# Amandaynzhou/MMT-PSM

Hardware: AMD Instinct MI355X
Metric: imgs/sec (student+teacher step, 1000x1000, AUG_K=2) (higher is better)
Workload: dtype f32

## Files before the change

mmt-psm_amd/csrc/conv_wgpl.hip:

```cpp
#include "conv_shared.h"

namespace {

constexpr unsigned WG_OOB = 0x80000000u;
constexpr int WG_BLK = 1024 + 128;
constexpr int WG_GSTAGE = 32 * WG_BLK;
constexpr int WG_STAGE = 2 * WG_GSTAGE, WG_S = 2;

typedef short s16x4 __attribute__((ext_vector_type(4)));

__device__ __forceinline__ f16x8 tr_pair(const char* p) {
  const s16x4 a = __builtin_amdgcn_ds_read_tr16_b64_v4i16((__attribute__((address_space(3))) s16x4*)(p));
  const s16x4 b = __builtin_amdgcn_ds_read_tr16_b64_v4i16((__attribute__((address_space(3))) s16x4*)(p + 128));
  typedef short s16x8 __attribute__((ext_vector_type(8)));
  const s16x8 v = {a[0], a[1], a[2], a[3], b[0], b[1], b[2], b[3]};
  return __builtin_bit_cast(f16x8, v);
}

struct WgP {
  const float* x; const float* dy;
  const unsigned short* xpl; long xpl_stride;
  const unsigned short* dpl; long dpl_stride;
  const float* s_x; const float* s_dy;
  const float* guard_x; const float* guard_dy;
  const float* rowscale; float* dw; float* ws; float* dbias;
  int N, H, W, Cin, Cout, KH, KW, pad, ksplit;
  int lag;
};

__device__ __forceinline__ void wgrad_pl_body(const WgP& p, const int bid_in, const int nwg_in) {
  extern __shared__ __attribute__((aligned(16))) float lds[];
  char* const ring = (char*)lds;
  const int tid = threadIdx.x, lane = tid & 63;
  const int wave = __builtin_amdgcn_readfirstlane(tid >> 6);
  const bool copier = wave >= 8;
  const int grp = copier ? (wave - 8) >> 1 : wave >> 2;
  const int gw = wave & 3, wm = gw >> 1, wn = gw & 1;
  const int NP = p.KH * p.KW * p.Cin, tiles_n = NP >> 7;
  int bid = bid_in;
  {
    const int nwg = nwg_in, q = nwg >> 3, r = nwg & 7, xcd = bid & 7, idx = bid >> 3;
    bid = (xcd < r ? xcd * (q + 1) : r * (q + 1) + (xcd - r) * q) + idx;
  }
  const int tile = bid % ((p.Cout >> 7) * tiles_n), ks = bid / ((p.Cout >> 7) * tiles_n);
  const int tile_m = tile / tiles_n, tile_n = tile - tile_m * tiles_n;
  const int co0 = tile_m * 128, n0 = tile_n * 128;
  const int tap = n0 / p.Cin, ci0 = n0 - tap * p.Cin;
  const int kh = tap / p.KW, kw = tap - kh * p.KW;
  const int dkh = kh - p.pad, dkw = kw - p.pad;
  const F16Guard gx = f16_guard_load(p.guard_x), gd = f16_guard_load(p.guard_dy);
  const int T = (p.N * p.H * p.W) >> 5, R = 2 * p.ksplit, rng = ks * 2 + grp;
  const int t0 = (int)((long)rng * T / R), nt = (int)((long)(rng + 1) * T / R) - t0;
  const int nt_max = (T + R - 1) / R;
  const int segs = p.W >> 5;
  char* const gring = ring + grp * WG_GSTAGE;

  f32x16 acc[2][2];
#pragma unroll
  for (int a = 0; a < 2; a++)
#pragma unroll
    for (int b = 0; b < 2; b++)
#pragma unroll
      for (int r = 0; r < 16; r++) acc[a][b][r] = 0.f;
  float bsum[2] = {0.f, 0.f};
  const bool do_bias = p.dbias != nullptr && tile_n == 0 && wn == 0 && !copier;
  const bool slow = ((p.lag & 1) ? f16_guard_bad_lag(gx, *p.s_x) : f16_guard_bad(gx)) ||
                    ((p.lag & 2) ? f16_guard_bad_lag(gd, *p.s_dy) : f16_guard_bad(gd));

  if (copier && !slow) {
    const int sub = (wave - 8) & 1;
    const long n_d = (long)p.N * p.H * p.W * p.Cout, n_x = (long)p.N * p.H * p.W * p.Cin;
    const __amdgpu_buffer_rsrc_t rs0 = sub == 0 ? __builtin_amdgcn_make_buffer_rsrc((void*)p.dpl, 0, (int)(n_d * 2), 0x00020000)
                                                : __builtin_amdgcn_make_buffer_rsrc((void*)((const char*)p.xpl - 64), 0, (int)(n_x * 2 + 64), 0x00020000);
    const __amdgpu_buffer_rsrc_t rs1 = sub == 0 ? __builtin_amdgcn_make_buffer_rsrc((void*)(p.dpl + p.dpl_stride), 0, (int)(n_d * 2), 0x00020000)
                                                : __builtin_amdgcn_make_buffer_rsrc((void*)((const char*)(p.xpl + p.xpl_stride) - 64), 0, (int)(n_x * 2 + 64), 0x00020000);
    const int cbn = (sub == 0 ? p.Cout : p.Cin) >> 4;
    const int cb0 = (sub == 0 ? co0 : ci0) >> 4;
    const int px = lane >> 1;
    int f_t = 0;
    auto copy_step = [&](int stage) {
      const bool real = f_t < nt;
      const int t = t0 + (real ? f_t : 0);
      const int row = t / segs, w0 = (t - row * segs) << 5;
      unsigned vo = (unsigned)lane * 16u;
      int soff;
      if (sub == 0) {
        soff = (row * cbn + cb0) * (p.W * 32) + w0 * 32;
        if (!real) vo = WG_OOB;
      } else {
        const int h = row % p.H, ih = h + dkh, iw = w0 + px + dkw;
        const bool ok = real && (unsigned)ih < (unsigned)p.H && (unsigned)iw < (unsigned)p.W;
        soff = ((row + dkh) * cbn + cb0) * (p.W * 32) + (w0 + dkw) * 32 + 64;
        if (!ok) { vo = WG_OOB; }
        if (!(real && (unsigned)ih < (unsigned)p.H)) soff = 64;
      }
      char* const st = gring + stage * WG_STAGE + sub * 16 * WG_BLK;
#pragma unroll
      for (int cb = 0; cb < 8; cb++) {
        __builtin_amdgcn_raw_ptr_buffer_load_lds(rs0, (lds_ptr_t)(st + cb * WG_BLK), 16, (int)vo, soff + cb * (p.W * 32), 0, 0);
        __builtin_amdgcn_raw_ptr_buffer_load_lds(rs1, (lds_ptr_t)(st + (8 + cb) * WG_BLK), 16, (int)vo, soff + cb * (p.W * 32), 0, 0);
      }
      f_t++;
    };
    copy_step(0);
    asm volatile("s_waitcnt vmcnt(0)" ::: "memory");
    __builtin_amdgcn_s_barrier();
    copy_step(1);
    for (int t = 0; t < nt_max; t++) {
      asm volatile("s_waitcnt vmcnt(0)" ::: "memory");
      __builtin_amdgcn_s_barrier();
      copy_step(t & 1);
    }
    asm volatile("s_waitcnt vmcnt(0)" ::: "memory");
  } else if (!slow) {
    const int i16 = lane & 15, g1 = (lane >> 4) & 1, khalf = lane >> 5;
    const int loff = khalf * 256 + (i16 >> 2) * 32 + (i16 & 3) * 8;
    const char* const fA = gring + (wm * 4 + g1) * WG_BLK + loff;
    const char* const fB = gring + (16 + wn * 4 + g1) * WG_BLK + loff;
    __builtin_amdgcn_s_barrier();
    for (int t = 0; t < nt_max; t++) {
      const char* const sa = fA + (t & 1) * WG_STAGE;
      const char* const sb = fB + (t & 1) * WG_STAGE;
      if (t < nt) {
#pragma unroll
        for (int k2 = 0; k2 < 2; k2++) {
          f16x8 fa[2][2], fb[2][2];
#pragma unroll
          for (int q = 0; q < 2; q++)
#pragma unroll
            for (int a = 0; a < 2; a++) {
              fa[q][a] = tr_pair(sa + (q * 8 + a * 2) * WG_BLK + k2 * 512);
              fb[q][a] = tr_pair(sb + (q * 8 + a * 2) * WG_BLK + k2 * 512);
            }
          if (do_bias) {
#pragma unroll
            for (int a = 0; a < 2; a++)
#pragma unroll
              for (int e = 0; e < 8; e++) bsum[a] += (float)fa[0][a][e] + (float)fa[1][a][e];
          }
#pragma unroll
          for (int pr = 0; pr < 3; pr++) {
            const int qa = pr == 1 ? 1 : 0, qb = pr == 0 ? 1 : 0;
#pragma unroll
            for (int a = 0; a < 2; a++)
#pragma unroll
              for (int b = 0; b < 2; b++) acc[a][b] = __builtin_amdgcn_mfma_f32_32x32x16_f16(fa[qa][a], fb[qb][b], acc[a][b], 0, 0, 0);
          }
        }
      }
      asm volatile("s_waitcnt lgkmcnt(0)" ::: "memory");
      __builtin_amdgcn_s_barrier();
    }
  }
  const float sxy = *p.s_x * *p.s_dy;
  if (slow) {
    if (!copier) {
      const int HW = p.H * p.W;
      for (int m = t0 * 32; m < (t0 + nt) * 32; m++) {
        const int img = m / HW, rem = m - img * HW, h = rem / p.W, w = rem - h * p.W;
        const int ih = h + dkh, iw = w + dkw;
        const bool ok = (unsigned)ih < (unsigned)p.H && (unsigned)iw < (unsigned)p.W;
#pragma unroll
        for (int b = 0; b < 2; b++) {
          const float xv = ok ? p.x[((long)(img * p.H + ih) * p.W + iw) * p.Cin + ci0 + wn * 64 + b * 32 + (lane & 31)] : 0.f;
#pragma unroll
          for (int a = 0; a < 2; a++)
#pragma unroll
            for (int r = 0; r < 16; r++) {
              const int co = co0 + wm * 64 + a * 32 + 8 * (r >> 2) + (r & 3) + 4 * (lane >> 5);
              acc[a][b][r] = fmaf(p.dy[(long)m * p.Cout + co], xv, acc[a][b][r]);
            }
        }
        if (do_bias && lane < 32) {
#pragma unroll
          for (int a = 0; a < 2; a++) bsum[a] += p.dy[(long)m * p.Cout + co0 + wm * 64 + a * 32 + lane] * *p.s_dy;
        }
      }
#pragma unroll
      for (int a = 0; a < 2; a++)
#pragma unroll
        for (int b = 0; b < 2; b++)
#pragma unroll
          for (int r = 0; r < 16; r++) acc[a][b][r] *= sxy;
    }
  }
  __syncthreads();

  if (do_bias) {
    const float inv_d = 1.f / *p.s_dy;
#pragma unroll
    for (int a = 0; a < 2; a++) {
      float v = bsum[a];
      if (!slow) v += __shfl_xor(v, 32, 64);
      if (lane < 32) atomicAdd(p.dbias + co0 + wm * 64 + a * 32 + lane, v * inv_d);
    }
  }

  {
    f32x4* const xch = (f32x4*)ring;
    const int gtid = tid & 255;
#pragma unroll
    for (int i = 0; i < 4; i++) {
      if (!copier && (i & 1) != grp) {
#pragma unroll
        for (int r4 = 0; r4 < 4; r4++)
          xch[(i * 4 + r4) * 256 + gtid] = f32x4{acc[i >> 1][i & 1][4 * r4], acc[i >> 1][i & 1][4 * r4 + 1],
                                                 acc[i >> 1][i & 1][4 * r4 + 2], acc[i >> 1][i & 1][4 * r4 + 3]};
      }
    }
    __syncthreads();
#pragma unroll
    for (int i = 0; i < 4; i++) {
      if (!copier && (i & 1) == grp) {
#pragma unroll
        for (int r4 = 0; r4 < 4; r4++) {
          const f32x4 v = xch[(i * 4 + r4) * 256 + gtid];
#pragma unroll
          for (int c = 0; c < 4; c++) {
            const float mine = acc[i >> 1][i & 1][4 * r4 + c];
            acc[i >> 1][i & 1][4 * r4 + c] = grp == 0 ? mine + v[c] : v[c] + mine;
          }
        }
      }
    }
  }
  if (copier) return;

  const float inv = 1.f / sxy;
  float* const dst = p.ksplit > 1 ? p.ws + (long)ks * p.Cout * NP : p.dw;
#pragma unroll
  for (int i = 0; i < 4; i++) {
    if ((i & 1) != grp) continue;
    const int a = i >> 1, b = i & 1;
#pragma unroll
    for (int r = 0; r < 16; r++) {
      const int co = co0 + wm * 64 + a * 32 + 8 * (r >> 2) + (r & 3) + 4 * (lane >> 5);
      float* const q = dst + (long)co * NP + n0 + wn * 64 + b * 32 + (lane & 31);
      if (p.ksplit > 1) *q = acc[a][b][r] * inv;
      else *q = *q + acc[a][b][r] * ((p.rowscale ? p.rowscale[co] : 1.f) * inv);
    }
  }
}

__global__ __launch_bounds__(768) void wgrad_pl_kernel(const WgP p) { wgrad_pl_body(p, blockIdx.x, gridDim.x); }

constexpr int WG_MAXG = 12;
struct WgGroup { WgP it[WG_MAXG]; int first[WG_MAXG + 1]; int n; };
static_assert(sizeof(WgGroup) <= 3584, "kernel-argument segment");
__global__ __launch_bounds__(768) void wgrad_pl_group_kernel(const WgGroup g) {
  int i = 0;
  for (int k = 1; k < g.n; k++) i = (int)blockIdx.x >= g.first[k] ? k : i;
  const int local = (int)blockIdx.x - g.first[i];
  const WgP p = g.it[i];
  const int real = (p.Cout >> 7) * ((p.KH * p.KW * p.Cin) >> 7) * p.ksplit;
  if (local >= real) return;
  wgrad_pl_body(p, local, real);
}

constexpr int WG_MAXR = 24;
struct WgReduceGroup { mmtconv::WgReduceItem it[WG_MAXR]; int first[WG_MAXR + 1]; int n; };
static_assert(sizeof(WgReduceGroup) <= 3584, "kernel-argument segment");
__global__ __launch_bounds__(256) void wgrad_reduce_group_kernel(const WgReduceGroup g) {
  int k = 0;
  for (int j = 1; j < g.n; j++) k = (int)blockIdx.x >= g.first[j] ? j : k;
  const mmtconv::WgReduceItem it = g.it[k];
  const int nb = g.first[k + 1] - g.first[k], lb = (int)blockIdx.x - g.first[k];
  const long n4 = (long)it.Cout * it.NP / 4, slab = (long)it.Cout * it.NP;
  for (long i = (long)lb * 256 + threadIdx.x; i < n4; i += (long)nb * 256) {
    f32x4 o = ((f32x4*)it.dw)[i];
    f32x4 a = ((const f32x4*)it.ws)[i];
    int s = 1;
    for (; s + 8 <= it.splits; s += 8) {
      f32x4 b[8];
#pragma unroll
      for (int u = 0; u < 8; u++) b[u] = *(const f32x4*)(it.ws + (s + u) * slab + i * 4);
#pragma unroll
      for (int u = 0; u < 8; u++) a += b[u];
    }
    for (; s < it.splits; s++) a += *(const f32x4*)(it.ws + s * slab + i * 4);
    const float sc = it.rowscale ? it.rowscale[(int)((i * 4) / it.NP)] : 1.f;
#pragma unroll
    for (int e = 0; e < 4; e++) o[e] += a[e] * sc;
    ((f32x4*)it.dw)[i] = o;
  }
}

__global__ __launch_bounds__(256) void wgrad_pl_reduce_kernel(const float* __restrict__ ws, int splits, int Cout, int NP,
                                                              const float* __restrict__ rowscale, float* __restrict__ dw) {
  const long n4 = (long)Cout * NP / 4, slab = (long)Cout * NP;
  for (long i = (long)blockIdx.x * 256 + threadIdx.x; i < n4; i += (long)gridDim.x * 256) {
    f32x4 o = ((f32x4*)dw)[i];
    f32x4 a = ((const f32x4*)ws)[i];
    int s = 1;
    for (; s + 8 <= splits; s += 8) {
      f32x4 b[8];
#pragma unroll
      for (int u = 0; u < 8; u++) b[u] = *(const f32x4*)(ws + (s + u) * slab + i * 4);
#pragma unroll
      for (int u = 0; u < 8; u++) a += b[u];
    }
    for (; s < splits; s++) a += *(const f32x4*)(ws + s * slab + i * 4);
    const float sc = rowscale ? rowscale[(int)((i * 4) / NP)] : 1.f;
#pragma unroll
    for (int e = 0; e < 4; e++) o[e] += a[e] * sc;
    ((f32x4*)dw)[i] = o;
  }
}

int wgpl_splits(const mmt_conv_args* a) {
  if (precision() != 3 || a->stride != 1 || a->Ho != a->H || a->Wo != a->W || (a->W & 31) || (a->Cin & 127) || (a->Cout & 127) ||
      a->KH != a->KW || a->pad != (a->KH - 1) / 2 || !(a->KH & 1) || a->N < 1 || a->io_bf16 ||
      (long)a->N * a->H * a->W * (a->Cin > a->Cout ? a->Cin : a->Cout) >= (1L << 29))
    return 0;
  const char* e = getenv("MMT_WGRAD_PLANES");
  if (e && atoi(e) == 0) return 0;
  const long T = ((long)a->N * a->H * a->W) >> 5;
  const long tiles = (long)(a->Cout >> 7) * ((long)a->KH * a->KW * a->Cin >> 7);
  constexpr long target = 256;
  long ks = target / tiles;
  if (ks > T / 8) ks = T / 8;
  if (ks < 1) ks = 1;
  if (T < 2) return 0;
  return (int)ks;
}

}

namespace mmtconv {
int wgpl_eligible_splits(const mmt_conv_args* a) { return a ? wgpl_splits(a) : 0; }
long wgpl_super_steps(const mmt_conv_args* a) { return ((long)a->N * a->H * a->W) >> 5; }

int launch_wgrad_reduce_group(const WgReduceItem* items, int n, hipStream_t s) {
  for (int i0 = 0; i0 < n; i0 += WG_MAXR) {
    WgReduceGroup g;
    g.n = n - i0 < WG_MAXR ? n - i0 : WG_MAXR;
    int nb = 0;
    for (int i = 0; i < g.n; i++) {
      g.it[i] = items[i0 + i];
      g.first[i] = nb;
      long b = ((long)items[i0 + i].Cout * items[i0 + i].NP / 4 + 255) / 256;
      nb += (int)(b > 1024 ? 1024 : b);
    }
    g.first[g.n] = nb;
    hipLaunchKernelGGL(wgrad_reduce_group_kernel, dim3(nb), dim3(256), 0, s, g);
    MMT_LAUNCH_CHECK();
  }
  return 0;
}

int launch_wgpl_group(const WgPlJob* jobs, int n, hipStream_t s) {
  if (n < 1 || n > WG_MAXG) return MMT_EINVAL;
  WgGroup g;
  g.n = n;
  int nb = 0;
  for (int i = 0; i < n; i++) {
    const WgPlJob& j = jobs[i];
    const mmt_conv_args* a = j.a;
    if (!a->x || !j.dy || !j.xpl || !j.dpl || !j.s_x || !j.s_dy || !j.dw || ((size_t)j.xpl & 15) || ((size_t)j.dpl & 15) ||
        (j.xpl_stride & 7) || (j.dpl_stride & 7) || j.ksplit < 1 || (j.ksplit > 1 && !j.ws))
      return MMT_EINVAL;
    WgP& p = g.it[i];
    p.x = a->x; p.dy = j.dy;
    p.xpl = (const unsigned short*)j.xpl; p.xpl_stride = j.xpl_stride;
    p.dpl = (const unsigned short*)j.dpl; p.dpl_stride = j.dpl_stride;
    p.s_x = j.s_x; p.s_dy = j.s_dy;
    p.guard_x = (const float*)a->f16_guard_x; p.guard_dy = (const float*)a->f16_guard_dy;
    p.rowscale = j.rowscale; p.dw = j.dw; p.ws = j.ws; p.dbias = j.dbias;
    p.lag = a->x_planes_lag;
    p.N = a->N; p.H = a->H; p.W = a->W; p.Cin = a->Cin; p.Cout = a->Cout; p.KH = a->KH; p.KW = a->KW; p.pad = a->pad; p.ksplit = j.ksplit;
    g.first[i] = nb;
    const int blocks = (a->Cout >> 7) * ((a->KH * a->KW * a->Cin) >> 7) * j.ksplit;
    nb += (blocks + 7) & ~7;
  }
  g.first[n] = nb;
  constexpr size_t lds = (size_t)WG_S * WG_STAGE;
  static bool done = false;
  if (!done) {
    const hipError_t e = hipFuncSetAttribute((const void*)wgrad_pl_group_kernel, hipFuncAttributeMaxDynamicSharedMemorySize, (int)lds);
    if (e != hipSuccess) return (int)e;
    done = true;
  }
  hipLaunchKernelGGL(wgrad_pl_group_kernel, dim3(nb), dim3(768), lds, s, g);
  MMT_LAUNCH_CHECK();
  return 0;
}
}

extern "C" int mmt_conv_wgrad_planes_splits(const mmt_conv_args* a) { return a ? wgpl_splits(a) : 0; }

extern "C" int mmt_conv_wgrad_planes(const mmt_conv_args* a, const float* dy, const void* x_planes, long x_plane_stride,
                                     const void* dy_planes, long dy_plane_stride, const float* s_x, const float* s_dy,
                                     const float* rowscale, float* dw, float* dbias, float* workspace, void* stream) {
  if (!a) return MMT_EINVAL;
  const int ks = wgpl_splits(a);
  if (ks == 0) return 1;
  if (!a->x || !dy || !x_planes || !dy_planes || !s_x || !s_dy || !dw || ((size_t)x_planes & 15) || ((size_t)dy_planes & 15) ||
      (x_plane_stride & 7) || (dy_plane_stride & 7) || (ks > 1 && !workspace))
    return MMT_EINVAL;
  WgP p;
  p.x = a->x; p.dy = dy;
  p.xpl = (const unsigned short*)x_planes; p.xpl_stride = x_plane_stride;
  p.dpl = (const unsigned short*)dy_planes; p.dpl_stride = dy_plane_stride;
  p.s_x = s_x; p.s_dy = s_dy;
  p.guard_x = (const float*)a->f16_guard_x; p.guard_dy = (const float*)a->f16_guard_dy;
  p.rowscale = rowscale; p.dw = dw; p.ws = workspace; p.dbias = dbias;
  p.lag = a->x_planes_lag;
  p.N = a->N; p.H = a->H; p.W = a->W; p.Cin = a->Cin; p.Cout = a->Cout; p.KH = a->KH; p.KW = a->KW; p.pad = a->pad; p.ksplit = ks;
  const int NP = a->KH * a->KW * a->Cin;
  const int tiles = (a->Cout >> 7) * (NP >> 7);
  constexpr size_t lds = (size_t)WG_S * WG_STAGE;
  static_assert(lds <= 160 * 1024 && lds >= 16 * 256 * 16, "LDS");
  static bool done = false;
  if (!done) {
    const hipError_t e = hipFuncSetAttribute((const void*)wgrad_pl_kernel, hipFuncAttributeMaxDynamicSharedMemorySize, (int)lds);
    if (e != hipSuccess) return (int)e;
    done = true;
  }
  hipStream_t s = (hipStream_t)stream;
  hipLaunchKernelGGL(wgrad_pl_kernel, dim3(tiles * ks), dim3(768), lds, s, p);
  MMT_LAUNCH_CHECK();
  if (ks > 1) {
    const long n4 = (long)a->Cout * NP / 4;
    int blocks = (int)((n4 + 255) / 256);
    if (blocks > 4096) blocks = 4096;
    hipLaunchKernelGGL(wgrad_pl_reduce_kernel, dim3(blocks), dim3(256), 0, s, workspace, ks, a->Cout, NP, rowscale, dw);
    MMT_LAUNCH_CHECK();
  }
  return 0;
}
```

mmt-psm_amd/csrc/conv_wgrad.hip:

```cpp
#include <stdlib.h>
#include <type_traits>
#include "conv_shared.h"

namespace {

template <bool FAST>
__global__ __launch_bounds__(256) void conv_wgrad_kernel(const ConvP p, const float* __restrict__ dy,
                                                         const float* __restrict__ rowscale,
                                                         float* __restrict__ dw, int m_per_split,
                                                         float* __restrict__ ws) {
  constexpr int BM = 128, BN = 128;
  extern __shared__ __attribute__((aligned(16))) float lds[];
  float* ldsA = lds;
  float* ldsB = lds + 2 * 32 * 128;
  const int tid = threadIdx.x, lane = tid & 63;
  const int wave = __builtin_amdgcn_readfirstlane(tid >> 6);
  const int wm = wave >> 1, wn = wave & 1;
  const int co0 = blockIdx.y * BM, n0 = blockIdx.x * BN;
  const int NP = p.KH * p.KW * p.Cin;
  const int ms = blockIdx.z * m_per_split;
  const int me = min(p.M, ms + m_per_split);
  if (ms >= me) return;

  const int c4 = tid & 31;
// ... 725 lines not shown
  for (long i = (long)blockIdx.x * 256 + threadIdx.x; i < n4; i += (long)gridDim.x * 256) {
    f32x4 o = ((f32x4*)dw)[i];
    f32x4 a = ((const f32x4*)ws)[i];
    int s = 1;
    for (; s + 8 <= splits; s += 8) {
      f32x4 b[8];
#pragma unroll
      for (int u = 0; u < 8; u++) b[u] = *(const f32x4*)(ws + (s + u) * slab + i * 4);
#pragma unroll
      for (int u = 0; u < 8; u++) a += b[u];
    }
    for (; s < splits; s++) a += *(const f32x4*)(ws + s * slab + i * 4);
    const float sc = (rowscale ? rowscale[(int)((i * 4) / NP)] : 1.f) * f16_inv;
#pragma unroll
    for (int e = 0; e < 4; e++) o[e] += a[e] * sc;
    ((f32x4*)dw)[i] = o;
  }
}

__global__ __launch_bounds__(256) void colsum_kernel(const float* __restrict__ dy, int M, int C,
                                                     float* __restrict__ out, int rows_per_block) {
  const int c = blockIdx.x * 64 + (threadIdx.x & 63);
  const int sub = threadIdx.x >> 6;
  const int r0 = blockIdx.y * rows_per_block, r1 = min(M, r0 + rows_per_block);
  float s = 0.f;
  if (c < C)
    for (int r = r0 + sub; r < r1; r += 4) s += dy[(long)r * C + c];
  __shared__ float red[4][64];
  red[sub][threadIdx.x & 63] = s;
  __syncthreads();
  if (sub == 0 && c < C) atomicAdd(out + c, red[0][threadIdx.x] + red[1][threadIdx.x] + red[2][threadIdx.x] + red[3][threadIdx.x]);
}

}

extern "C" int mmt_conv_wgrad_splits(const mmt_conv_args* a) {
  ConvP p;
  int e = fill(p, a);
  if (e) return e;
  if (p.M == 0 || p.Cout == 0) return 1;
  const int NP = p.KH * p.KW * p.Cin;
  const int tx = mmt_cdiv(NP, 128), ty = mmt_cdiv(p.Cout, 128);
  const long tiles = (long)tx * ty;
  constexpr int slots = 512;
  constexpr int min_px = 512;
  int split = (int)(tiles >= slots ? 1 : slots / tiles);
  const int max_split = mmt_cdiv(p.M, min_px);
  if (split > max_split) split = max_split;
  if (split < 1) split = 1;
  int mps = mmt_cdiv(p.M, split);
  mps = (mps + 31) / 32 * 32;
  return mmt_cdiv(p.M, mps);
}

extern "C" int mmt_conv_wgrad(const mmt_conv_args* a, const float* dy, const float* rowscale, float* dw,
                              float* dbias, float* workspace, void* stream) {
  ConvP p;
  int e = fill(p, a);
  if (e) return e;
  if (!dy || !dw || !p.cin4) return MMT_EINVAL;
  if (p.M == 0 || p.Cout == 0) return 0;
  hipStream_t s = (hipStream_t)stream;
  const int NP = p.KH * p.KW * p.Cin;
  const int tx = mmt_cdiv(NP, 128), ty = mmt_cdiv(p.Cout, 128);
  const int split = mmt_conv_wgrad_splits(a);
  int mps = mmt_cdiv(p.M, split);
  mps = (mps + 31) / 32 * 32;
  if (split > 1 && !workspace) return MMT_EINVAL;
  float* ws = split > 1 ? workspace : nullptr;
  const bool fast = (p.Cout & 3) == 0 && p.Wo >= 8 && p.Ho >= 8;
  const int prec = precision();
  const int bf = ((p.io & IO_X) ? 1 : 0) | ((p.io & IO_DY) ? 2 : 0);
  const bool f16 = a->f16_x_amax && a->f16_dy_amax;
  if (f16) {
    if (prec != 3 || bf || (p.Cout & 3) || (mps & 15) || !((long)p.N * p.H * p.W * p.Cin * 4 < (1L << 31) && (long)p.M * p.Cout * 4 < (1L << 31)))
      return MMT_EINVAL;
    p.f16_sx = (const float*)a->f16_x_amax;
    p.f16_sw = (const float*)a->f16_dy_amax;
    const dim3 grid(tx, ty, split);
    const int mode = !(p.Wo >= 8 && p.Ho >= 8) ? 0 : ((p.Wo & 3) == 0 ? 2 : 1);
#define WGF(MODE) hipLaunchKernelGGL((conv_wgrad_pipe_kernel<2, MODE, true, 0, true>), grid, dim3(256), (size_t)65536, s, p, dy, rowscale, dw, mps, ws, dbias)
    if (mode == 2) WGF(2); else if (mode == 1) WGF(1); else WGF(0);
#undef WGF
    MMT_LAUNCH_CHECK();
    if (split > 1) {
      const long n4 = (long)p.Cout * NP / 4;
      int blocks = (int)((n4 + 255) / 256);
      if (blocks > 4096) blocks = 4096;
      hipLaunchKernelGGL(wgrad_reduce_kernel, dim3(blocks), dim3(256), 0, s, ws, split, p.Cout, NP, rowscale, dw);
      MMT_LAUNCH_CHECK();
    }
    return 0;
  }
  if (bf && !(prec == 1 && (p.Cout & 3) == 0 && (mps & 15) == 0 && (long)p.N * p.H * p.W * p.Cin * 4 < (1L << 31) &&
              (long)p.M * p.Cout * 4 < (1L << 31)))
    return MMT_EINVAL;
  constexpr int pipe_any = 1;
  const bool small_t = (long)p.N * p.H * p.W * p.Cin * 4 < (1L << 31) && (long)p.M * p.Cout * 4 < (1L << 31);
  if (prec > 0 && ((p.Cout & 3) == 0 || (pipe_any && small_t)) && (mps & 15) == 0) {
    const dim3 grid(tx, ty, split);
    constexpr int pipe = 1;
    const bool small = (long)p.N * p.H * p.W * p.Cin * 4 < (1L << 31) && (long)p.M * p.Cout * 4 < (1L << 31);
    const int mode = !(p.Wo >= 8 && p.Ho >= 8) ? 0 : ((p.Wo & 3) == 0 ? 2 : 1);
    const bool vec4 = (p.Cout & 3) == 0;
    const size_t wg_lds = prec >= 3 ? 73728 : 65536;
#define WGPL(K) do { if (wg_lds > 65536) { const hipError_t er = hipFuncSetAttribute((const void*)K, hipFuncAttributeMaxDynamicSharedMemorySize, (int)wg_lds); if (er != hipSuccess) return (int)er; } hipLaunchKernelGGL(K, grid, dim3(256), wg_lds, s, p, dy, rowscale, dw, mps, ws, dbias); } while (0)
#define WGP(NS, MODE) do { if (bf && NS == 1) { if (bf == 1) WGPL((conv_wgrad_pipe_kernel<1, MODE, true, 1>)); else if (bf == 2) WGPL((conv_wgrad_pipe_kernel<1, MODE, true, 2>)); else WGPL((conv_wgrad_pipe_kernel<1, MODE, true, 3>)); } else if (vec4) WGPL((conv_wgrad_pipe_kernel<NS, MODE, true>)); else WGPL((conv_wgrad_pipe_kernel<NS, MODE, false>)); } while (0)
#define WGP3(NS) do { if (mode == 2) WGP(NS, 2); else if (mode == 1) WGP(NS, 1); else WGP(NS, 0); } while (0)
#define WGS(NS, INC) do { if ((pipe && small) || bf) WGP3(NS); else hipLaunchKernelGGL((conv_wgrad_split_kernel<NS, INC>), grid, dim3(256), (size_t)65536, s, p, dy, rowscale, dw, mps, ws, dbias); } while (0)
    if (fast) { if (prec == 1) WGS(1, true); else if (prec == 2) WGS(2, true); else WGS(3, true); }
    else { if (prec == 1) WGS(1, false); else if (prec == 2) WGS(2, false); else WGS(3, false); }
#undef WGP3
#undef WGP
#undef WGPL
#undef WGS
    dbias = nullptr;
  } else if (fast)
    hipLaunchKernelGGL(conv_wgrad_kernel<true>, dim3(tx, ty, split), dim3(256), (size_t)4 * 4096 * sizeof(float), s, p,
                       dy, rowscale, dw, mps, ws);
  else
    hipLaunchKernelGGL(conv_wgrad_kernel<false>, dim3(tx, ty, split), dim3(256), (size_t)4 * 4096 * sizeof(float), s, p,
                       dy, rowscale, dw, mps, ws);
  MMT_LAUNCH_CHECK();
  if (split > 1) {
    const long n4 = (long)p.Cout * NP / 4;
    int blocks = (int)((n4 + 255) / 256);
    if (blocks > 4096) blocks = 4096;
    hipLaunchKernelGGL(wgrad_reduce_kernel, dim3(blocks), dim3(256), 0, s, ws, split, p.Cout, NP, rowscale, dw);
    MMT_LAUNCH_CHECK();
  }
  if (dbias) {
    int rpb = 1024;
    hipLaunchKernelGGL(colsum_kernel, dim3(mmt_cdiv(p.Cout, 64), mmt_cdiv(p.M, rpb)), dim3(256), 0, s, dy, p.M,
                       p.Cout, dbias, rpb);
    MMT_LAUNCH_CHECK();
  }
  return 0;
}

namespace {
constexpr int WG_CAP_PL = 12, WG_CAP_PIPE = WGP_MAXG;
struct WgJobPlan { int kind; int split; int mps; long ws_off; };
constexpr int WGJ_MAX = 96;

static bool wg_job_pipe_ok(const mmt_wgrad_job& j, ConvP& p) {
  if (fill(p, &j.a) || !j.dy || !j.dw || !p.cin4 || p.M == 0 || p.Cout == 0) return false;
  if (!j.a.f16_x_amax || !j.a.f16_dy_amax || precision() != 3 || p.io || (p.Cout & 3)) return false;
  return (long)p.N * p.H * p.W * p.Cin * 4 < (1L << 31) && (long)p.M * p.Cout * 4 < (1L << 31);
}

static long wg_plan(const mmt_wgrad_job* jobs, int n, WgJobPlan* plan) {
  const char* e = getenv("MMT_WGRAD_GROUP");
  const bool on = !(e && atoi(e) == 0);
  constexpr int WG_DIV = 4;
  int kind[WGJ_MAX];
  for (int i = 0; i < n; i++) {
    ConvP p;
    kind[i] = 0;
    if (on && jobs[i].x_planes && jobs[i].dy_planes && wgpl_eligible_splits(&jobs[i].a) > 0) kind[i] = 1;
    else if (on && wg_job_pipe_ok(jobs[i], p)) kind[i] = 2 + (!(p.Wo >= 8 && p.Ho >= 8) ? 0 : ((p.Wo & 3) == 0 ? 2 : 1));
  }
  for (int i = 1; i < n; i++)
    for (int j = 0; j < i; j++)
      if (jobs[j].dw == jobs[i].dw || (jobs[i].dbias && jobs[j].dbias == jobs[i].dbias)) { kind[i] = 0; break; }
  for (int k = 1; k <= 4; k++) {
    int cnt = 0, last = -1;
    for (int i = 0; i < n; i++) if (kind[i] == k) { cnt++; last = i; }
    if (cnt == 1) kind[last] = 0;
  }
  long ws = 0;
  for (int k = 1; k <= 4; k++)
    for (int i = 0; i < n; i++) {
      if (kind[i] != k) continue;
      const mmt_conv_args& a = jobs[i].a;
      const int NP = a.KH * a.KW * a.Cin;
      WgJobPlan& pl = plan[i];
      pl.kind = k; pl.mps = 0;
      if (k == 1) {
        long ks = (wgpl_eligible_splits(&a) + WG_DIV - 1) / WG_DIV;
        const long T = wgpl_super_steps(&a);
        if (ks > T / 8) ks = T / 8;
        if (ks < 1) ks = 1;
        pl.split = (int)ks;
      } else {
        const int M = a.N * a.Ho * a.Wo;
        long sp = (mmt_conv_wgrad_splits(&a) + WG_DIV - 1) / WG_DIV;
        const long mx = mmt_cdiv(M, 512);
        if (sp > mx) sp = mx;
        if (sp < 1) sp = 1;
        int mps = mmt_cdiv(M, (int)sp);
        mps = (mps + 31) / 32 * 32;
        pl.mps = mps;
        pl.split = mmt_cdiv(M, mps);
      }
      pl.ws_off = ws;
      if (pl.split > 1) ws += (long)pl.split * a.Cout * NP;
    }
  for (int i = 0; i < n; i++) {
    if (kind[i] != 0) continue;
    WgJobPlan& pl = plan[i];
    const mmt_conv_args& a = jobs[i].a;
    pl.kind = 0; pl.mps = 0;
    int sp = 0;
    if (jobs[i].x_planes && jobs[i].dy_planes) sp = wgpl_eligible_splits(&a);
    if (sp <= 0) sp = mmt_conv_wgrad_splits(&a);
    pl.split = sp < 1 ? 1 : sp;
    pl.ws_off = ws;
    if (pl.split > 1) ws += (long)pl.split * a.Cout * a.KH * a.KW * a.Cin;
  }
  return ws;
}
}

extern "C" int mmt_conv_wgrad_group_workspace(const mmt_wgrad_job* jobs, int n, long* floats_out) {
  if (!jobs || !floats_out || n < 0 || n > WGJ_MAX) return MMT_EINVAL;
  WgJobPlan plan[WGJ_MAX];
  *floats_out = wg_plan(jobs, n, plan);
  return 0;
}

extern "C" int mmt_conv_wgrad_group(const mmt_wgrad_job* jobs, int n, float* workspace, long workspace_floats, void* stream) {
  if (!jobs || n < 0 || n > WGJ_MAX) return MMT_EINVAL;
  if (n == 0) return 0;
  WgJobPlan plan[WGJ_MAX];
  const long need = wg_plan(jobs, n, plan);
  if (need > 0 && (!workspace || workspace_floats < need)) return MMT_EINVAL;
  hipStream_t s = (hipStream_t)stream;
  WgReduceItem red[WGJ_MAX];
  int nred = 0;
  {
    WgPlJob g[WG_CAP_PL];
    int m = 0;
    auto flush = [&]() -> int {
      if (m == 0) return 0;
      const int e = launch_wgpl_group(g, m, s);
      m = 0;
      return e;
    };
    for (int i = 0; i < n; i++) {
      if (plan[i].kind != 1) continue;
      const mmt_wgrad_job& j = jobs[i];
      float* ws = plan[i].split > 1 ? workspace + plan[i].ws_off : nullptr;
      g[m++] = WgPlJob{&j.a, j.dy, j.x_planes, j.x_plane_stride, j.dy_planes, j.dy_plane_stride, j.s_x, j.s_dy, j.rowscale, j.dw, j.dbias, ws,
                       plan[i].split};
      if (plan[i].split > 1)
        red[nred++] = WgReduceItem{ws, j.rowscale, j.dw, plan[i].split, j.a.Cout, j.a.KH * j.a.KW * j.a.Cin, 0};
      if (m == WG_CAP_PL) { const int e = flush(); if (e) return e; }
    }
    const int e = flush();
    if (e) return e;
  }
  for (int mode = 0; mode < 3; mode++) {
    WgPipeGroup g;
    g.n = 0;
    int nb = 0;
    auto flush = [&]() -> int {
      if (g.n == 0) return 0;
      g.first[g.n] = nb;
      if (mode == 2) hipLaunchKernelGGL(conv_wgrad_pipe_group_kernel<2>, dim3(nb), dim3(256), (size_t)65536, s, g);
      else if (mode == 1) hipLaunchKernelGGL(conv_wgrad_pipe_group_kernel<1>, dim3(nb), dim3(256), (size_t)65536, s, g);
      else hipLaunchKernelGGL(conv_wgrad_pipe_group_kernel<0>, dim3(nb), dim3(256), (size_t)65536, s, g);
      g.n = 0;
      nb = 0;
      MMT_LAUNCH_CHECK();
      return 0;
    };
    for (int i = 0; i < n; i++) {
      if (plan[i].kind != 2 + mode) continue;
      const mmt_wgrad_job& j = jobs[i];
      WgPipeItem& it = g.it[g.n];
      if (!wg_job_pipe_ok(j, it.p) || (plan[i].mps & 15)) return MMT_EINVAL;
      it.p.f16_sx = (const float*)j.a.f16_x_amax;
      it.p.f16_sw = (const float*)j.a.f16_dy_amax;
      const int NP = it.p.KH * it.p.KW * it.p.Cin;
      it.dy = j.dy; it.rowscale = j.rowscale; it.dw = j.dw; it.dbias = j.dbias;
      it.ws = plan[i].split > 1 ? workspace + plan[i].ws_off : nullptr;
      it.mps = plan[i].mps; it.tx = mmt_cdiv(NP, 128); it.ty = mmt_cdiv(it.p.Cout, 128); it.tz = plan[i].split;
      if (plan[i].split > 1) red[nred++] = WgReduceItem{it.ws, j.rowscale, j.dw, plan[i].split, it.p.Cout, NP, 0};
      g.first[g.n] = nb;
      nb += (it.tx * it.ty * it.tz + 7) & ~7;
      g.n++;
      if (g.n == WG_CAP_PIPE) { const int e = flush(); if (e) return e; }
    }
    const int e = flush();
    if (e) return e;
  }
  if (nred) { const int e = launch_wgrad_reduce_group(red, nred, s); if (e) return e; }
  for (int i = 0; i < n; i++) {
    if (plan[i].kind != 0) continue;
    const mmt_wgrad_job& j = jobs[i];
    float* ws = plan[i].split > 1 ? workspace + plan[i].ws_off : nullptr;
    int e = 1;
    if (j.x_planes && j.dy_planes)
      e = mmt_conv_wgrad_planes(&j.a, j.dy, j.x_planes, j.x_plane_stride, j.dy_planes, j.dy_plane_stride, j.s_x, j.s_dy, j.rowscale, j.dw,
                                j.dbias, ws, stream);
    if (e == 1) e = mmt_conv_wgrad(&j.a, j.dy, j.rowscale, j.dw, j.dbias, ws, stream);
    if (e) return e;
  }
  return 0;
}

extern "C" int mmt_colsum(const float* dy, int M, int C, float* out, void* stream) {
  if (M <= 0 || C <= 0) return 0;
  const int rpb = 1024;
  hipLaunchKernelGGL(colsum_kernel, dim3(mmt_cdiv(C, 64), mmt_cdiv(M, rpb)), dim3(256), 0, (hipStream_t)stream, dy, M,
                     C, out, rpb);
  MMT_LAUNCH_CHECK();
  return 0;
}
```

Before: 127.9.

## Add 3-tap row-reuse form of plane wgrad kernel with deeper LDS pipeline

Result: faster. 130.4, median of 6 (+1.9%).

```diff
diff --git a/mmt-psm_amd/csrc/conv_wgpl.hip b/mmt-psm_amd/csrc/conv_wgpl.hip
--- a/mmt-psm_amd/csrc/conv_wgpl.hip
+++ b/mmt-psm_amd/csrc/conv_wgpl.hip
@@ -5,7 +5,18 @@
 constexpr unsigned WG_OOB = 0x80000000u;
 constexpr int WG_BLK = 1024 + 128;
 constexpr int WG_GSTAGE = 32 * WG_BLK;
-constexpr int WG_STAGE = 2 * WG_GSTAGE, WG_S = 2;
+
+template <int TAPS> struct WgForm {
+  static constexpr int NG = TAPS == 1 ? 2 : 1;
+  static constexpr int WN = 4 / NG;
+  static constexpr int NB = 4 / WN;
+  static constexpr int STAGE = NG * WG_GSTAGE;
+  static constexpr int S = TAPS == 1 ? 2 : 4;
+  static constexpr int PER = TAPS == 1 ? 16 : 12;
+  static constexpr size_t LDS = (size_t)S * STAGE;
+  static_assert(LDS <= 160 * 1024 && LDS >= 16 * 256 * 16, "LDS");
+  static_assert((S - 2) * PER < 64, "vmcnt");
+};
 
 typedef short s16x4 __attribute__((ext_vector_type(4)));
 
@@ -15,6 +26,12 @@
   typedef short s16x8 __attribute__((ext_vector_type(8)));
   const s16x8 v = {a[0], a[1], a[2], a[3], b[0], b[1], b[2], b[3]};
   return __builtin_bit_cast(f16x8, v);
+}
+
+template <int N> __device__ __forceinline__ void wait_vm() {
+  static_assert(N == 0 || N == 24, "vmcnt");
+  if (N == 0) asm volatile("s_waitcnt vmcnt(0)" ::: "memory");
+  else asm volatile("s_waitcnt vmcnt(24)" ::: "memory");
 }
 
 struct WgP {
@@ -28,15 +45,19 @@
   int lag;
 };
 
-__device__ __forceinline__ void wgrad_pl_body(const WgP& p, const int bid_in, const int nwg_in) {
+__host__ __device__ __forceinline__ int wg_tiles_n(int KH, int KW, int Cin) { return (KW == 3 ? KH * Cin : KH * KW * Cin) >> 7; }
+
+template <int TAPS> __device__ __forceinline__ void wgrad_pl_body(const WgP& p, const int bid_in, const int nwg_in) {
+  typedef WgForm<TAPS> F;
+  constexpr int NG = F::NG, WN = F::WN, NB = F::NB, NJ = NB * TAPS;
   extern __shared__ __attribute__((aligned(16))) float lds[];
   char* const ring = (char*)lds;
   const int tid = threadIdx.x, lane = tid & 63;
   const int wave = __builtin_amdgcn_readfirstlane(tid >> 6);
   const bool copier = wave >= 8;
-  const int grp = copier ? (wave - 8) >> 1 : wave >> 2;
-  const int gw = wave & 3, wm = gw >> 1, wn = gw & 1;
-  const int NP = p.KH * p.KW * p.Cin, tiles_n = NP >> 7;
+  const int grp = NG == 1 ? 0 : (copier ? (wave - 8) >> 1 : wave >> 2);
+  const int gw = wave & (8 / NG - 1), wm = gw / WN, wn = gw % WN;
+  const int NP = p.KH * p.KW * p.Cin, tiles_n = wg_tiles_n(p.KH, p.KW, p.Cin);
   int bid = bid_in;
   {
     const int nwg = nwg_in, q = nwg >> 3, r = nwg & 7, xcd = bid & 7, idx = bid >> 3;
@@ -44,94 +65,118 @@
   }
   const int tile = bid % ((p.Cout >> 7) * tiles_n), ks = bid / ((p.Cout >> 7) * tiles_n);
   const int tile_m = tile / tiles_n, tile_n = tile - tile_m * tiles_n;
-  const int co0 = tile_m * 128, n0 = tile_n * 128;
-  const int tap = n0 / p.Cin, ci0 = n0 - tap * p.Cin;
-  const int kh = tap / p.KW, kw = tap - kh * p.KW;
+  const int co0 = tile_m * 128;
+  int n0, kh, kw, ci0;
+  if (TAPS == 1) {
+    n0 = tile_n * 128;
+    const int tap = n0 / p.Cin;
+    ci0 = n0 - tap * p.Cin; kh = tap / p.KW; kw = tap - kh * p.KW;
+  } else {
+    kh = (tile_n * 128) / p.Cin; ci0 = tile_n * 128 - kh * p.Cin; kw = 0;
+    n0 = kh * TAPS * p.Cin + ci0;
+  }
   const int dkh = kh - p.pad, dkw = kw - p.pad;
   const F16Guard gx = f16_guard_load(p.guard_x), gd = f16_guard_load(p.guard_dy);
-  const int T = (p.N * p.H * p.W) >> 5, R = 2 * p.ksplit, rng = ks * 2 + grp;
+  const int T = (p.N * p.H * p.W) >> 5, R = NG * p.ksplit, rng = ks * NG + grp;
   const int t0 = (int)((long)rng * T / R), nt = (int)((long)(rng + 1) * T / R) - t0;
   const int nt_max = (T + R - 1) / R;
   const int segs = p.W >> 5;
   char* const gring = ring + grp * WG_GSTAGE;
 
-  f32x16 acc[2][2];
+  f32x16 acc[2][NJ];
 #pragma unroll
   for (int a = 0; a < 2; a++)
 #pragma unroll
-    for (int b = 0; b < 2; b++)
-#pragma unroll
-      for (int r = 0; r < 16; r++) acc[a][b][r] = 0.f;
+    for (int j = 0; j < NJ; j++)
+#pragma unroll
+      for (int r = 0; r < 16; r++) acc[a][j][r] = 0.f;
   float bsum[2] = {0.f, 0.f};
   const bool do_bias = p.dbias != nullptr && tile_n == 0 && wn == 0 && !copier;
   const bool slow = ((p.lag & 1) ? f16_guard_bad_lag(gx, *p.s_x) : f16_guard_bad(gx)) ||
                     ((p.lag & 2) ? f16_guard_bad_lag(gd, *p.s_dy) : f16_guard_bad(gd));
 
   if (copier && !slow) {
-    const int sub = (wave - 8) & 1;
+    const int sub = (wave - 8) & 1, hb = TAPS == 1 ? 0 : (wave - 8) >> 1;
     const long n_d = (long)p.N * p.H * p.W * p.Cout, n_x = (long)p.N * p.H * p.W * p.Cin;
-    const __amdgpu_buffer_rsrc_t rs0 = sub == 0 ? __builtin_amdgcn_make_buffer_rsrc((void*)p.dpl, 0, (int)(n_d * 2), 0x00020000)
-                                                : __builtin_amdgcn_make_buffer_rsrc((void*)((const char*)p.xpl - 64), 0, (int)(n_x * 2 + 64), 0x00020000);
-    const __amdgpu_buffer_rsrc_t rs1 = sub == 0 ? __builtin_amdgcn_make_buffer_rsrc((void*)(p.dpl + p.dpl_stride), 0, (int)(n_d * 2), 0x00020000)
-                                                : __builtin_amdgcn_make_buffer_rsrc((void*)((const char*)(p.xpl + p.xpl_stride) - 64), 0, (int)(n_x * 2 + 64), 0x00020000);
-    const int cbn = (sub == 0 ? p.Cout : p.Cin) >> 4;
-    const int cb0 = (sub == 0 ? co0 : ci0) >> 4;
+    const int q0 = TAPS == 1 ? 0 : sub, q1 = TAPS == 1 ? 1 : sub;
+    const bool isA = TAPS == 1 && sub == 0, isB = TAPS == 1 && sub == 1;
+    const __amdgpu_buffer_rsrc_t rsd = isB ? __builtin_amdgcn_make_buffer_rsrc((void*)((const char*)(p.xpl + q0 * p.xpl_stride) - 64), 0, (int)(n_x * 2 + 64), 0x00020000)
+                                           : __builtin_amdgcn_make_buffer_rsrc((void*)(p.dpl + q0 * p.dpl_stride), 0, (int)(n_d * 2), 0x00020000);
+    const __amdgpu_buffer_rsrc_t rsx = isA ? __builtin_amdgcn_make_buffer_rsrc((void*)(p.dpl + q1 * p.dpl_stride), 0, (int)(n_d * 2), 0x00020000)
+                                           : __builtin_amdgcn_make_buffer_rsrc((void*)((const char*)(p.xpl + q1 * p.xpl_stride) - 64), 0, (int)(n_x * 2 + 64), 0x00020000);
+    const int cbn_d = p.Cout >> 4, cbn_x = p.Cin >> 4;
+    const int cb0_d = (co0 >> 4) + hb * 4, cb0_x = (ci0 >> 4) + hb * 4;
     const int px = lane >> 1;
     int f_t = 0;
     auto copy_step = [&](int stage) {
       const bool real = f_t < nt;
       const int t = t0 + (real ? f_t : 0);
       const int row = t / segs, w0 = (t - row * segs) << 5;
-      unsigned vo = (unsigned)lane * 16u;
-      int soff;
-      if (sub == 0) {
-        soff = (row * cbn + cb0) * (p.W * 32) + w0 * 32;
-        if (!real) vo = WG_OOB;
+      const unsigned vo_d = real ? (unsigned)lane * 16u : WG_OOB;
+      const int so_d = (row * cbn_d + cb0_d) * (p.W * 32) + w0 * 32;
+      const int h = row % p.H, ih = h + dkh, iw = w0 + px + dkw;
+      const bool rowok = real && (unsigned)ih < (unsigned)p.H;
+      const unsigned vo_x = rowok && (unsigned)iw < (unsigned)p.W ? (unsigned)lane * 16u : WG_OOB;
+      const int so_x = rowok ? ((row + dkh) * cbn_x + cb0_x) * (p.W * 32) + (w0 + dkw) * 32 + 64 : 64;
+      if (TAPS == 1) {
+        char* const st = gring + stage * F::STAGE + sub * 16 * WG_BLK;
+        const unsigned vo = sub == 0 ? vo_d : vo_x;
+        const int so = sub == 0 ? so_d : so_x, cs = p.W * 32;
+#pragma unroll
+        for (int cb = 0; cb < 8; cb++) {
+          __builtin_amdgcn_raw_ptr_buffer_load_lds(rsd, (lds_ptr_t)(st + cb * WG_BLK), 16, (int)vo, so + cb * cs, 0, 0);
+          __builtin_amdgcn_raw_ptr_buffer_load_lds(rsx, (lds_ptr_t)(st + (8 + cb) * WG_BLK), 16, (int)vo, so + cb * cs, 0, 0);
+        }
       } else {
-        const int h = row % p.H, ih = h + dkh, iw = w0 + px + dkw;
-        const bool ok = real && (unsigned)ih < (unsigned)p.H && (unsigned)iw < (unsigned)p.W;
-        soff = ((row + dkh) * cbn + cb0) * (p.W * 32) + (w0 + dkw) * 32 + 64;
-        if (!ok) { vo = WG_OOB; }
-        if (!(real && (unsigned)ih < (unsigned)p.H)) soff = 64;
-      }
-      char* const st = gring + stage * WG_STAGE + sub * 16 * WG_BLK;
-#pragma unroll
-      for (int cb = 0; cb < 8; cb++) {
-        __builtin_amdgcn_raw_ptr_buffer_load_lds(rs0, (lds_ptr_t)(st + cb * WG_BLK), 16, (int)vo, soff + cb * (p.W * 32), 0, 0);
-        __builtin_amdgcn_raw_ptr_buffer_load_lds(rs1, (lds_ptr_t)(st + (8 + cb) * WG_BLK), 16, (int)vo, soff + cb * (p.W * 32), 0, 0);
+        char* const st = gring + stage * F::STAGE + (sub * 8 + hb * 4) * WG_BLK;
+        const int cs = p.W * 32;
+#pragma unroll
+        for (int cb = 0; cb < 4; cb++) {
+          __builtin_amdgcn_raw_ptr_buffer_load_lds(rsd, (lds_ptr_t)(st + cb * WG_BLK), 16, (int)vo_d, so_d + cb * cs, 0, 0);
+          __builtin_amdgcn_raw_ptr_buffer_load_lds(rsx, (lds_ptr_t)(st + (16 + cb) * WG_BLK), 16, (int)vo_x, so_x + cb * cs, 0, 0);
+        }
+        if (lane < 4) {
+          const unsigned vo_t = rowok && w0 + 32 + px + dkw < p.W ? 1024u + (unsigned)lane * 16u : WG_OOB;
+#pragma unroll
+          for (int cb = 0; cb < 4; cb++)
+            __builtin_amdgcn_raw_ptr_buffer_load_lds(rsx, (lds_ptr_t)(st + (16 + cb) * WG_BLK + 1024), 16, (int)vo_t, so_x + cb * cs, 0, 0);
+        }
       }
       f_t++;
     };
-    copy_step(0);
-    asm volatile("s_waitcnt vmcnt(0)" ::: "memory");
+#pragma unroll
+    for (int u = 0; u < F::S - 1; u++) copy_step(u);
+    wait_vm<(F::S - 2) * F::PER>();
     __builtin_amdgcn_s_barrier();
-    copy_step(1);
     for (int t = 0; t < nt_max; t++) {
-      asm volatile("s_waitcnt vmcnt(0)" ::: "memory");
+      copy_step((t + F::S - 1) & (F::S - 1));
+      wait_vm<(F::S - 2) * F::PER>();
       __builtin_amdgcn_s_barrier();
-      copy_step(t & 1);
-    }
-    asm volatile("s_waitcnt vmcnt(0)" ::: "memory");
+    }
+    wait_vm<0>();
   } else if (!slow) {
     const int i16 = lane & 15, g1 = (lane >> 4) & 1, khalf = lane >> 5;
     const int loff = khalf * 256 + (i16 >> 2) * 32 + (i16 & 3) * 8;
     const char* const fA = gring + (wm * 4 + g1) * WG_BLK + loff;
-    const char* const fB = gring + (16 + wn * 4 + g1) * WG_BLK + loff;
+    const char* const fB = gring + (16 + wn * 2 * NB + g1) * WG_BLK + loff;
     __builtin_amdgcn_s_barrier();
     for (int t = 0; t < nt_max; t++) {
-      const char* const sa = fA + (t & 1) * WG_STAGE;
-      const char* const sb = fB + (t & 1) * WG_STAGE;
+      const char* const sa = fA + (t & (F::S - 1)) * F::STAGE;
+      const char* const sb = fB + (t & (F::S - 1)) * F::STAGE;
       if (t < nt) {
 #pragma unroll
         for (int k2 = 0; k2 < 2; k2++) {
-          f16x8 fa[2][2], fb[2][2];
-#pragma unroll
-          for (int q = 0; q < 2; q++)
-#pragma unroll
-            for (int a = 0; a < 2; a++) {
-              fa[q][a] = tr_pair(sa + (q * 8 + a * 2) * WG_BLK + k2 * 512);
-              fb[q][a] = tr_pair(sb + (q * 8 + a * 2) * WG_BLK + k2 * 512);
-            }
+          f16x8 fa[2][2], fb[2][NJ];
+#pragma unroll
+          for (int q = 0; q < 2; q++) {
+#pragma unroll
+            for (int a = 0; a < 2; a++) fa[q][a] = tr_pair(sa + (q * 8 + a * 2) * WG_BLK + k2 * 512);
+#pragma unroll
+            for (int b = 0; b < NB; b++)
+#pragma unroll
+              for (int k = 0; k < TAPS; k++)
+                fb[q][b * TAPS + k] = tr_pair(sb + (q * 8 + b * 2) * WG_BLK + k2 * 512 + k * 32);
+          }
           if (do_bias) {
 #pragma unroll
             for (int a = 0; a < 2; a++)
@@ -144,7 +189,7 @@
 #pragma unroll
             for (int a = 0; a < 2; a++)
 #pragma unroll
-              for (int b = 0; b < 2; b++) acc[a][b] = __builtin_amdgcn_mfma_f32_32x32x16_f16(fa[qa][a], fb[qb][b], acc[a][b], 0, 0, 0);
+              for (int j = 0; j < NJ; j++) acc[a][j] = __builtin_amdgcn_mfma_f32_32x32x16_f16(fa[qa][a], fb[qb][j], acc[a][j], 0, 0, 0);
           }
         }
       }
@@ -158,17 +203,18 @@
       const int HW = p.H * p.W;
       for (int m = t0 * 32; m < (t0 + nt) * 32; m++) {
         const int img = m / HW, rem = m - img * HW, h = rem / p.W, w = rem - h * p.W;
-        const int ih = h + dkh, iw = w + dkw;
-        const bool ok = (unsigned)ih < (unsigned)p.H && (unsigned)iw < (unsigned)p.W;
-#pragma unroll
-        for (int b = 0; b < 2; b++) {
-          const float xv = ok ? p.x[((long)(img * p.H + ih) * p.W + iw) * p.Cin + ci0 + wn * 64 + b * 32 + (lane & 31)] : 0.f;
+        const int ih = h + dkh;
+#pragma unroll
+        for (int j = 0; j < NJ; j++) {
+          const int b = j / TAPS, iw = w + dkw + j % TAPS;
+          const bool ok = (unsigned)ih < (unsigned)p.H && (unsigned)iw < (unsigned)p.W;
+          const float xv = ok ? p.x[((long)(img * p.H + ih) * p.W + iw) * p.Cin + ci0 + wn * (32 * NB) + b * 32 + (lane & 31)] : 0.f;
 #pragma unroll
           for (int a = 0; a < 2; a++)
 #pragma unroll
             for (int r = 0; r < 16; r++) {
               const int co = co0 + wm * 64 + a * 32 + 8 * (r >> 2) + (r & 3) + 4 * (lane >> 5);
-              acc[a][b][r] = fmaf(p.dy[(long)m * p.Cout + co], xv, acc[a][b][r]);
+              acc[a][j][r] = fmaf(p.dy[(long)m * p.Cout + co], xv, acc[a][j][r]);
             }
         }
         if (do_bias && lane < 32) {
@@ -179,9 +225,9 @@
 #pragma unroll
       for (int a = 0; a < 2; a++)
 #pragma unroll
-        for (int b = 0; b < 2; b++)
-#pragma unroll
-          for (int r = 0; r < 16; r++) acc[a][b][r] *= sxy;
+        for (int j = 0; j < NJ; j++)
+#pragma unroll
+          for (int r = 0; r < 16; r++) acc[a][j][r] *= sxy;
     }
   }
   __syncthreads();
@@ -196,29 +242,29 @@
     }
   }
 
-  {
+  if constexpr (NG == 2) {
     f32x4* const xch = (f32x4*)ring;
     const int gtid = tid & 255;
 #pragma unroll
-    for (int i = 0; i < 4; i++) {
+    for (int i = 0; i < 2 * NJ; i++) {
       if (!copier && (i & 1) != grp) {
 #pragma unroll
         for (int r4 = 0; r4 < 4; r4++)
-          xch[(i * 4 + r4) * 256 + gtid] = f32x4{acc[i >> 1][i & 1][4 * r4], acc[i >> 1][i & 1][4 * r4 + 1],
-                                                 acc[i >> 1][i & 1][4 * r4 + 2], acc[i >> 1][i & 1][4 * r4 + 3]};
+          xch[(i * 4 + r4) * 256 + gtid] = f32x4{acc[i / NJ][i % NJ][4 * r4], acc[i / NJ][i % NJ][4 * r4 + 1],
+                                                 acc[i / NJ][i % NJ][4 * r4 + 2], acc[i / NJ][i % NJ][4 * r4 + 3]};
       }
     }
     __syncthreads();
 #pragma unroll
-    for (int i = 0; i < 4; i++) {
+    for (int i = 0; i < 2 * NJ; i++) {
       if (!copier && (i & 1) == grp) {
 #pragma unroll
         for (int r4 = 0; r4 < 4; r4++) {
           const f32x4 v = xch[(i * 4 + r4) * 256 + gtid];
 #pragma unroll
           for (int c = 0; c < 4; c++) {
-            const float mine = acc[i >> 1][i & 1][4 * r4 + c];
-            acc[i >> 1][i & 1][4 * r4 + c] = grp == 0 ? mine + v[c] : v[c] + mine;
+            const float mine = acc[i / NJ][i % NJ][4 * r4 + c];
+            acc[i / NJ][i % NJ][4 * r4 + c] = grp == 0 ? mine + v[c] : v[c] + mine;
           }
         }
       }
@@ -229,32 +275,36 @@
   const float inv = 1.f / sxy;
   float* const dst = p.ksplit > 1 ? p.ws + (long)ks * p.Cout * NP : p.dw;
 #pragma unroll
-  for (int i = 0; i < 4; i++) {
-    if ((i & 1) != grp) continue;
-    const int a = i >> 1, b = i & 1;
-#pragma unroll
-    for (int r = 0; r < 16; r++) {
-      const int co = co0 + wm * 64 + a * 32 + 8 * (r >> 2) + (r & 3) + 4 * (lane >> 5);
-      float* const q = dst + (long)co * NP + n0 + wn * 64 + b * 32 + (lane & 31);
-      if (p.ksplit > 1) *q = acc[a][b][r] * inv;
-      else *q = *q + acc[a][b][r] * ((p.rowscale ? p.rowscale[co] : 1.f) * inv);
-    }
-  }
-}
-
-__global__ __launch_bounds__(768) void wgrad_pl_kernel(const WgP p) { wgrad_pl_body(p, blockIdx.x, gridDim.x); }
+  for (int a = 0; a < 2; a++)
+#pragma unroll
+    for (int j = 0; j < NJ; j++) {
+      if (NG == 2 && (j & 1) != grp) continue;
+      const int b = j / TAPS, k = j % TAPS;
+#pragma unroll
+      for (int r = 0; r < 16; r++) {
+        const int co = co0 + wm * 64 + a * 32 + 8 * (r >> 2) + (r & 3) + 4 * (lane >> 5);
+        float* const q = dst + (long)co * NP + n0 + k * p.Cin + wn * (32 * NB) + b * 32 + (lane & 31);
+        if (p.ksplit > 1) *q = acc[a][j][r] * inv;
+        else *q = *q + acc[a][j][r] * ((p.rowscale ? p.rowscale[co] : 1.f) * inv);
+      }
+    }
+}
+
+template <int TAPS> __global__ __launch_bounds__(768) void wgrad_pl_kernel(const WgP p) { wgrad_pl_body<TAPS>(p, blockIdx.x, gridDim.x); }
 
 constexpr int WG_MAXG = 12;
 struct WgGroup { WgP it[WG_MAXG]; int first[WG_MAXG + 1]; int n; };
 static_assert(sizeof(WgGroup) <= 3584, "kernel-argument segment");
+static_assert(WgForm<1>::LDS == WgForm<3>::LDS, "one dynamic LDS size for both forms of a grouped launch");
 __global__ __launch_bounds__(768) void wgrad_pl_group_kernel(const WgGroup g) {
   int i = 0;
   for (int k = 1; k < g.n; k++) i = (int)blockIdx.x >= g.first[k] ? k : i;
   const int local = (int)blockIdx.x - g.first[i];
   const WgP p = g.it[i];
-  const int real = (p.Cout >> 7) * ((p.KH * p.KW * p.Cin) >> 7) * p.ksplit;
+  const int real = (p.Cout >> 7) * wg_tiles_n(p.KH, p.KW, p.Cin) * p.ksplit;
   if (local >= real) return;
-  wgrad_pl_body(p, local, real);
+  if (p.KW == 3) wgrad_pl_body<3>(p, local, real);
+  else wgrad_pl_body<1>(p, local, real);
 }
 
 constexpr int WG_MAXR = 24;
@@ -315,9 +365,9 @@
   const char* e = getenv("MMT_WGRAD_PLANES");
   if (e && atoi(e) == 0) return 0;
   const long T = ((long)a->N * a->H * a->W) >> 5;
-  const long tiles = (long)(a->Cout >> 7) * ((long)a->KH * a->KW * a->Cin >> 7);
-  constexpr long target = 256;
-  long ks = target / tiles;
+  const long tiles = (long)(a->Cout >> 7) * wg_tiles_n(a->KH, a->KW, a->Cin);
+  constexpr long target = 256, target3 = 256;
+  long ks = (a->KW == 3 ? target3 : target) / tiles;
   if (ks > T / 8) ks = T / 8;
   if (ks < 1) ks = 1;
   if (T < 2) return 0;
@@ -369,11 +419,11 @@
     p.lag = a->x_planes_lag;
     p.N = a->N; p.H = a->H; p.W = a->W; p.Cin = a->Cin; p.Cout = a->Cout; p.KH = a->KH; p.KW = a->KW; p.pad = a->pad; p.ksplit = j.ksplit;
     g.first[i] = nb;
-    const int blocks = (a->Cout >> 7) * ((a->KH * a->KW * a->Cin) >> 7) * j.ksplit;
+    const int blocks = (a->Cout >> 7) * wg_tiles_n(a->KH, a->KW, a->Cin) * j.ksplit;
     nb += (blocks + 7) & ~7;
   }
   g.first[n] = nb;
-  constexpr size_t lds = (size_t)WG_S * WG_STAGE;
+  constexpr size_t lds = WgForm<3>::LDS;
   static bool done = false;
   if (!done) {
     const hipError_t e = hipFuncSetAttribute((const void*)wgrad_pl_group_kernel, hipFuncAttributeMaxDynamicSharedMemorySize, (int)lds);
@@ -407,17 +457,19 @@
   p.lag = a->x_planes_lag;
   p.N = a->N; p.H = a->H; p.W = a->W; p.Cin = a->Cin; p.Cout = a->Cout; p.KH = a->KH; p.KW = a->KW; p.pad = a->pad; p.ksplit = ks;
   const int NP = a->KH * a->KW * a->Cin;
-  const int tiles = (a->Cout >> 7) * (NP >> 7);
-  constexpr size_t lds = (size_t)WG_S * WG_STAGE;
-  static_assert(lds <= 160 * 1024 && lds >= 16 * 256 * 16, "LDS");
-  static bool done = false;
-  if (!done) {
-    const hipError_t e = hipFuncSetAttribute((const void*)wgrad_pl_kernel, hipFuncAttributeMaxDynamicSharedMemorySize, (int)lds);
+  const int tiles = (a->Cout >> 7) * wg_tiles_n(a->KH, a->KW, a->Cin);
+  const bool kw3 = a->KW == 3;
+  const size_t lds = kw3 ? WgForm<3>::LDS : WgForm<1>::LDS;
+  static bool done[2] = {false, false};
+  if (!done[kw3]) {
+    const hipError_t e = hipFuncSetAttribute(kw3 ? (const void*)wgrad_pl_kernel<3> : (const void*)wgrad_pl_kernel<1>,
+                                             hipFuncAttributeMaxDynamicSharedMemorySize, (int)lds);
     if (e != hipSuccess) return (int)e;
-    done = true;
+    done[kw3] = true;
   }
   hipStream_t s = (hipStream_t)stream;
-  hipLaunchKernelGGL(wgrad_pl_kernel, dim3(tiles * ks), dim3(768), lds, s, p);
+  if (kw3) hipLaunchKernelGGL(wgrad_pl_kernel<3>, dim3(tiles * ks), dim3(768), lds, s, p);
+  else hipLaunchKernelGGL(wgrad_pl_kernel<1>, dim3(tiles * ks), dim3(768), lds, s, p);
   MMT_LAUNCH_CHECK();
   if (ks > 1) {
     const long n4 = (long)a->Cout * NP / 4;
diff --git a/mmt-psm_amd/csrc/conv_wgrad.hip b/mmt-psm_amd/csrc/conv_wgrad.hip
--- a/mmt-psm_amd/csrc/conv_wgrad.hip
+++ b/mmt-psm_amd/csrc/conv_wgrad.hip
@@ -901,7 +901,7 @@
 static long wg_plan(const mmt_wgrad_job* jobs, int n, WgJobPlan* plan) {
   const char* e = getenv("MMT_WGRAD_GROUP");
   const bool on = !(e && atoi(e) == 0);
-  constexpr int WG_DIV = 4;
+  constexpr int WG_DIV = 4, WG_DIV_PL = 4;
   int kind[WGJ_MAX];
   for (int i = 0; i < n; i++) {
     ConvP p;
@@ -926,7 +926,7 @@
       WgJobPlan& pl = plan[i];
       pl.kind = k; pl.mps = 0;
       if (k == 1) {
-        long ks = (wgpl_eligible_splits(&a) + WG_DIV - 1) / WG_DIV;
+        long ks = (wgpl_eligible_splits(&a) + WG_DIV_PL - 1) / WG_DIV_PL;
         const long T = wgpl_super_steps(&a);
         if (ks > T / 8) ks = T / 8;
         if (ks < 1) ks = 1;
```
